# erwincoumans/tiny-differentiable-simulator

Hardware: AMD Instinct MI355X
Metric: env-steps/sec (higher is better)
Workload: dtype f64

## Files before the change

### tiny-differentiable-simulator_amd/csrc/tds_oct.hip

```cpp
#include <hip/hip_runtime.h>
#include <stdlib.h>

#include "tds_device_model.h"
#include "tds_kernels.h"
#include "tds_lanes.h"
#include "tds_step_shared.h"

#ifdef TDS_OCT_PROF
#ifndef TDS_OCT_PROF_WG
#define TDS_OCT_PROF_WG 3
#endif
__device__ unsigned long long tds_oct_prof_buf[32];
__device__ unsigned long long tds_oct_prof_clk[64];
__device__ unsigned long long tds_oct_prof_wg[3 * 2048];
__device__ int tds_oct_prof_iter = 500;
#define OCT_STAMP(k, pin)                                                                       \
  do {                                                                                          \
    unsigned long long t_;                                                                      \
    auto p_ = (pin);        \
    asm volatile("s_memtime %0\n\ts_waitcnt lgkmcnt(0)" : "=s"(t_), "+v"(p_)::"memory");        \
    if (prof_on) prof_t[k] = t_;                                                                \
  } while (0)
#else
#define OCT_STAMP(k, pin) do { } while (0)
// ... 28 lines not shown
__device__ __forceinline__ T pair_other(T v) { return oct_dpp<0xB1>(v); }
template <int K, typename T>
__device__ __forceinline__ T pair_bcast(T v) { return oct_dpp<(K == 0 ? 0xA0 : 0xF5)>(v); }
template <typename T>
__device__ __forceinline__ T oct_sum(T v) {
  asm volatile("" : "+v"(v));
  v += oct_dpp<0xB1>(v);
  v += oct_dpp<0x4E>(v);
  v += oct_dpp<0x141>(v);
  return v;
}
template <int K>
__device__ __forceinline__ double oct_bcast(double v) {
  const double t = __builtin_amdgcn_update_dpp(0.0, v, 0x150 + K, 0xF, 0x3, false);
  return __builtin_amdgcn_update_dpp(t, v, 0x150 + 8 + K, 0xF, 0xC, false);
}
template <int K>
__device__ __forceinline__ float oct_bcast(float v) {
  const int b = __float_as_int(v);
  const int t = __builtin_amdgcn_update_dpp(0, b, 0x150 + K, 0xF, 0x3, false);
  return __int_as_float(__builtin_amdgcn_update_dpp(t, b, 0x150 + 8 + K, 0xF, 0xC, false));
}

struct OctOff {
  int lcw, legf, swl, qdp, fac, win, xs, cp, stride;
};
struct OctLds {
  static constexpr int LCW = 6;
  static constexpr int ZW = 14;
  static constexpr int Z_B = 10, Z_A = 11, Z_G = 12, Z_HL = 13;
  static constexpr int NCP = 17;
};
__host__ __device__ inline OctOff oct_layout(int in_dim) {
  OctOff o;
  int at = in_dim + 4;
  at = (at + 1) & ~1;
  o.lcw = at;  at += 8 * OctLds::LCW;
  o.legf = at; at += 4 * 3;
  o.swl = at;  at += 8 * 6;
  o.qdp = at;  at += 8;
  o.fac = at;  at += 28;
  o.win = at;  at += 2 * 8 * OctLds::ZW;
  o.xs = at;   at += 3 * OctLds::NCP + 1;
  o.cp = at;   at += 5 * OctLds::NCP + 1;
  at = (at + 1) & ~1;
  while ((((at * 2) & 63) % 8) != 0 || ((at * 2) & 63) == 0 || ((at * 2) & 63) == 32) at += 2;
  o.stride = at;
  return o;
}

struct OctKernArgs {
  const void *mdl, *x_in;
  void *y_out;
  const void *actions;
  void *x_feedback, *obs_out;
  TdsStepCtl ctl;
  int n_envs;
  OctOff O;
};
using TB = TdsOctTab;

#ifdef TDS_OCT_NT
#define OCT_ST(v, p) __builtin_nontemporal_store((v), (p))
// ... 93 lines not shown
    unsigned long long c0_, c1_;
    asm volatile("s_memtime %0\n\ts_memrealtime %1\n\ts_waitcnt lgkmcnt(0)" : "=s"(c0_), "=s"(c1_)::"memory");
    tds_oct_prof_clk[2 * it] = c0_;
    tds_oct_prof_clk[2 * it + 1] = c1_;
  }
#endif
  const int lane = tid & 7;
  const int grp = (tid & 63) >> 3;
  const int env = blockIdx.x * 8 + grp;
  const bool valid = env < n_envs;
  T *const E = sm + grp * O.stride;
  T *const xr = E;
  const int leg = lane >> 1, pos = lane & 1;
  const int dq = 6 + lane;
  const T *const CL = CT + lane * TB::LSTR;
  typename TdsCtlRef<LOOP>::type ctl = TdsCtlRef<LOOP>::get(ctl_arg, ka_seg + __builtin_offsetof(OctKernArgs, ctl));
  const T dt = CT[TB::SC + TB::DT];
  const int pgs_iters = (int)CT[TB::SC + TB::PGS_ITERATIONS];
  const bool last = it == nsteps - 1;
  OCT_STAMP(0, tid);

  T q, qd, tau;
  T Sl[6], R[9], p[3], sw[6], v[6], a0[6];
  T R5[9], P[3], A4[3], A5[3], pA3[3], pA4[3], pA5[3], v5[6], a5[6];
  T Lc[6], l10, id0, id1, sq0, sq1, my_id, my_sq, Ls[15], ids[6], sq_ids[6], qd_new, qdr_new[6];
  T Cb, Cr[6], It[10];
  T u = T(0), urm = T(0);
  T u_init = T(0), urm_init = T(0);
  int na = 0, NA = 0;

  auto root_frame = [&](T sx, T cx, T sy, T cy, T sz, T cz) {
    R5[0] = cy * cz;                 R5[1] = -cy * sz;                R5[2] = sy;
    R5[3] = sx * sy * cz + cx * sz;  R5[4] = cx * cz - sx * sy * sz;  R5[5] = -sx * cy;
    R5[6] = sx * sz - cx * sy * cz;  R5[7] = cx * sy * sz + sx * cz;  R5[8] = cx * cy;
    P[0] = xr[0] + CT[TB::SC + TB::BASE_T];
    P[1] = xr[1] + CT[TB::SC + TB::BASE_T + 1];
    P[2] = xr[2] + CT[TB::SC + TB::BASE_T + 2];
    A4[0] = T(0); A4[1] = cx; A4[2] = sx;
    A5[0] = sy; A5[1] = -sx * cy; A5[2] = cx * cy;
    pA3[0] = T(0); pA3[1] = P[2]; pA3[2] = -P[1];
    cross3(P, A4, pA4);
    cross3(P, A5, pA5);
  };
  auto times_inertia = [&](const T *I, const T *s, T *F) {
    T t3[3];
    sym3_mulv(I, s, F);
    cross3(I + 6, s + 3, t3);
    F[0] += t3[0];
    F[1] += t3[1];
    F[2] += t3[2];
    cross3(I + 6, s, t3);
    F[3] = I[9] * s[3] - t3[0];
    F[4] = I[9] * s[4] - t3[1];
    F[5] = I[9] * s[5] - t3[2];
  };
  auto dot6 = [&](const T *a, const T *b) -> T { return dot3(a, b) + dot3(a + 3, b + 3); };

  auto main_kin = [&]() {
    OCT_MARK("main_top");
    q = xr[dq];
    qd = xr[nq + dq];
    tau = T(0);
    {
      const int act_i = act_slot;
      if (act_i >= 0) {
        const int var = nq + nd + adim;
        const T kp = xr[var], kd = xr[var + 1], max_force = xr[var + 2];
        const T act_lim = CT[TB::SC + TB::ACTION_LIMIT];
        T a = xr[nq + nd + act_i];
        a = a < act_lim ? a : act_lim;
        a = a > -act_lim ? a : -act_lim;
        const T q_des = CL[TB::IPOSE] + a;
        T f = kp * (q_des - q) + kd * (T(0) - qd);
        f = f > -max_force ? f : -max_force;
        f = f < max_force ? f : max_force;
        tau = f;
      }
      tau -= CL[TB::STIFF] * q + CL[TB::DAMP] * qd;
      asm volatile("" : "+v"(tau));
    }
    OCT_MARK("main_jcalc");
#pragma unroll
    for (int k = 0; k < 6; ++k) Sl[k] = CL[TB::S + k];
    T Rp[9], tp[3];
    {
      T sn, cs;
      tds_sincos(q * CL[TB::ROTF], &sn, &cs);
      const T c1 = T(1) - cs;
      const T nx = CL[TB::NAX], ny = CL[TB::NAX + 1], nz = CL[TB::NAX + 2];
      T RJ[9];
      RJ[0] = cs + c1 * CL[TB::NN + 0];
      RJ[1] = c1 * CL[TB::NN + 1] - sn * nz;
      RJ[2] = c1 * CL[TB::NN + 2] + sn * ny;
      RJ[3] = c1 * CL[TB::NN + 1] + sn * nz;
      RJ[4] = cs + c1 * CL[TB::NN + 3];
      RJ[5] = c1 * CL[TB::NN + 4] - sn * nx;
      RJ[6] = c1 * CL[TB::NN + 2] - sn * ny;
      RJ[7] = c1 * CL[TB::NN + 4] + sn * nx;
      RJ[8] = cs + c1 * CL[TB::NN + 5];
      const T tJ[3] = {Sl[3] * q, Sl[4] * q, Sl[5] * q};
      if (CT[TB::SC + TB::XT_IDENT] != T(0)) {
#pragma unroll
        for (int k = 0; k < 9; ++k) Rp[k] = RJ[k];
#pragma unroll
        for (int k = 0; k < 3; ++k) tp[k] = CL[TB::XT + 9 + k] + tJ[k];
      } else {
        T RT[9], r[3];
#pragma unroll
        for (int k = 0; k < 9; ++k) RT[k] = CL[TB::XT + k];
        mat3_mul(RT, RJ, Rp);
        mat3_mulv(RT, tJ, r);
#pragma unroll
        for (int k = 0; k < 3; ++k) tp[k] = CL[TB::XT + 9 + k] + r[k];
      }
    }
    OCT_MARK("main_rootsincos");
    {
      T rs, rc;
      tds_sincos(xr[3 + (lane < 3 ? lane : 0)], &rs, &rc);
      const T sx = oct_bcast<0>(rs), cx = oct_bcast<0>(rc);
      const T sy = oct_bcast<1>(rs), cy = oct_bcast<1>(rc);
      const T sz = oct_bcast<2>(rs), cz = oct_bcast<2>(rc);
      if constexpr (W2) {
        if (lane < 3) {
          T *const sc = E + O.win + 8 * OctLds::ZW + 96;
          sc[2 * lane] = rs;
          sc[2 * lane + 1] = rc;
        }
      }
      root_frame(sx, cx, sy, cy, sz, cz);
    }
    OCT_MARK("main_rootvel");
    {
      const T d0 = xr[nq + 0], d1 = xr[nq + 1], d2 = xr[nq + 2], d3 = xr[nq + 3], d4 = xr[nq + 4], d5 = xr[nq + 5];
      const T U[3] = {d0, d1, d2};
      const T J3[3] = {d3, T(0), T(0)}, J4[3] = {A4[0] * d4, A4[1] * d4, A4[2] * d4}, J5[3] = {A5[0] * d5, A5[1] * d5, A5[2] * d5};
      const T W4[3] = {J3[0] + J4[0], J3[1] + J4[1], J3[2] + J4[2]};
      const T W5[3] = {W4[0] + J5[0], W4[1] + J5[1], W4[2] + J5[2]};
      T pJ3[3], pJ4[3], pJ5[3];
      cross3(P, J3, pJ3);
      cross3(P, J4, pJ4);
      cross3(P, J5, pJ5);
      const T pW4[3] = {pJ3[0] + pJ4[0], pJ3[1] + pJ4[1], pJ3[2] + pJ4[2]};
      const T pW5[3] = {pW4[0] + pJ5[0], pW4[1] + pJ5[1], pW4[2] + pJ5[2]};
      const T V3[3] = {U[0] + pJ3[0], U[1] + pJ3[1], U[2] + pJ3[2]};
      const T V4[3] = {U[0] + pW4[0], U[1] + pW4[1], U[2] + pW4[2]};
      const T V5[3] = {U[0] + pW5[0], U[1] + pW5[1], U[2] + pW5[2]};
      T a45[3], a55[3], t1[3], t2[3], l3[3], l4[3], l5[3];
      cross3(J3, J4, a45);
      cross3(W4, J5, a55);
      cross3(J3, pJ3, t1);
      cross3(V3, J3, t2);
      l3[0] = t1[0] + t2[0]; l3[1] = t1[1] + t2[1]; l3[2] = t1[2] + t2[2];
      cross3(W4, pJ4, t1);
      cross3(V4, J4, t2);
      l4[0] = t1[0] + t2[0]; l4[1] = t1[1] + t2[1]; l4[2] = t1[2] + t2[2];
      cross3(W5, pJ5, t1);
      cross3(V5, J5, t2);
      l5[0] = t1[0] + t2[0]; l5[1] = t1[1] + t2[1]; l5[2] = t1[2] + t2[2];
#pragma unroll
      for (int k = 0; k < 3; ++k) {
        v5[k] = W5[k];
        v5[3 + k] = V5[k];
        a5[k] = a45[k] + a55[k];
        a5[3 + k] = (l3[k] + l4[k] + l5[k]) - CT[TB::SC + TB::GRAV + k];
      }
    }
    OCT_MARK("main_legs");
    {
      const bool take = pos == 1;
      T Rq[9], pq[3];
#pragma unroll
      for (int k = 0; k < 9; ++k) {
        const T sh = pair_bcast<0>(Rp[k]);
        Rq[k] = take ? sh : ((k == 0 || k == 4 || k == 8) ? T(1) : T(0));
      }
#pragma unroll
      for (int k = 0; k < 3; ++k) {
        const T sh = pair_bcast<0>(tp[k]);
        pq[k] = take ? sh : T(0);
      }
      T Rl[9], pl[3], r[3];
      mat3_mul(Rq, Rp, Rl);
      mat3_mulv(Rq, tp, r);
#pragma unroll
      for (int k = 0; k < 3; ++k) pl[k] = pq[k] + r[k];
      mat3_mul(R5, Rl, R);
      mat3_mulv(R5, pl, r);
      p[0] = P[0] + r[0];
      p[1] = P[1] + r[1];
      p[2] = P[2] + r[2];
      mat3_mulv(R, Sl, sw);
      mat3_mulv(R, Sl + 3, sw + 3);
      T c[3];
      cross3(p, sw, c);
      sw[3] += c[0];
      sw[4] += c[1];
      sw[5] += c[2];
      T vJ[6];
#pragma unroll
      for (int k = 0; k < 6; ++k) vJ[k] = sw[k] * qd;
#pragma unroll
      for (int k = 0; k < 6; ++k) {
        const T sh = pair_bcast<0>(vJ[k]);
        v[k] = v5[k] + (vJ[k] + (take ? sh : T(0)));
      }
      T cb[6];
      cross3(v, vJ, cb);
      T c1[3], c2[3];
      cross3(v, vJ + 3, c1);
      cross3(v + 3, vJ, c2);
      cb[3] = c1[0] + c2[0];
      cb[4] = c1[1] + c2[1];
      cb[5] = c1[2] + c2[2];
#pragma unroll
      for (int k = 0; k < 6; ++k) {
        const T sh = pair_bcast<0>(cb[k]);
        a0[k] = a5[k] + (cb[k] + (take ? sh : T(0)));
      }
    }
    OCT_MARK("main_publish_kin");
    {
      T *const swl = E + O.swl + lane * 6;
#pragma unroll
      for (int k = 0; k < 6; ++k) swl[k] = sw[k];
      if constexpr (W2) {
        T *const kin = E + O.win + 8 * OctLds::ZW + lane * 12;
#pragma unroll
        for (int k = 0; k < 9; ++k) kin[k] = R[k];
#pragma unroll
        for (int k = 0; k < 3; ++k) kin[9 + k] = p[k];
      }
    }
    OCT_MARK("main_kin_end");
    OCT_STAMP(1, sw[5]);
  };

// ... 20 lines not shown
  auto help_np = [&]() {
    OCT_MARK("help_np");
    if constexpr (LOOP) {
      if (it > 0 && ctl.obs_ring != nullptr && ctl.peer_arrive != nullptr)
        sig_tok = tds_peer_count_in(ctl, (o_slot == 0 ? ctl.obs_slots : o_slot) - 1);
      if (ctl.act_pool != nullptr && it + 1 < nsteps && valid)
        next_act = (T)tds_global((const TR *)ctl.act_pool)[((size_t)act_blk * ctl.act_envs + env) * adim + lane];
    }
    if constexpr (W2) {
      const T *const kin = E + O.win + 8 * OctLds::ZW + lane * 12;
#pragma unroll
      for (int k = 0; k < 9; ++k) R[k] = kin[k];
#pragma unroll
      for (int k = 0; k < 3; ++k) p[k] = kin[9 + k];
      const T *const sc = E + O.win + 8 * OctLds::ZW + 96;
      root_frame(sc[0], sc[1], sc[2], sc[3], sc[4], sc[5]);
    }
    {
      T *const cpx = E + O.cp;
      const T n[3] = {CT[TB::SC + TB::PLANE_N], CT[TB::SC + TB::PLANE_N + 1], CT[TB::SC + TB::PLANE_N + 2]};
      const T pc = CT[TB::SC + TB::PLANE_C];
      auto sphere = [&](const T *Rl, const T *pl, const T *loc, T rad, T *pt, T &dist) {
        T ctr[3];
        mat3_mulv(Rl, loc, ctr);
        ctr[0] += pl[0];
        ctr[1] += pl[1];
        ctr[2] += pl[2];
        const T t = -((-dot3(ctr, n)) + pc);
        dist = t - rad;
        pt[0] = ctr[0] - rad * n[0];
        pt[1] = ctr[1] - rad * n[1];
        pt[2] = ctr[2] - rad * n[2];
      };
      T pt0[3], pt1[3], ptt[3], d0, d1, dtt;
      sphere(R, p, CL + TB::CPL0, CL[TB::CPR0], pt0, d0);
      sphere(R, p, CL + TB::CPL1, CL[TB::CPR1], pt1, d1);
      sphere(R5, P, CT + TB::ROOT + TB::R_CPL, CT[TB::ROOT + TB::R_CPR], ptt, dtt);
      const bool act0 = valid && d0 < T(0), act1 = valid && d1 < T(0), actt = valid && dtt < T(0) && CT[TB::ROOT + TB::R_CPR] >= T(0);
      const unsigned long long b0 = __ballot(act0), b1 = __ballot(act1), bt = __ballot(actt);
      const unsigned m0 = (unsigned)((b0 >> (grp * 8)) & 0xFFull), m1 = (unsigned)((b1 >> (grp * 8)) & 0xFFull);
      const unsigned below = (1u << lane) - 1u;
      const int r0 = (actt ? 1 : 0) + __popc(m0 & below) + __popc(m1 & below);
      const int r1 = r0 + (act0 ? 1 : 0);
      if (act0) {
        cpx[0 * OctLds::NCP + r0] = pt0[0];
        cpx[1 * OctLds::NCP + r0] = pt0[1];
        cpx[2 * OctLds::NCP + r0] = pt0[2];
        cpx[3 * OctLds::NCP + r0] = d0;
        cpx[4 * OctLds::NCP + r0] = (T)lane;
      }
// ... 3 lines not shown
        cpx[2 * OctLds::NCP + r1] = pt1[2];
        cpx[3 * OctLds::NCP + r1] = d1;
        cpx[4 * OctLds::NCP + r1] = (T)lane;
      }
      if (actt && lane == 0) {
        cpx[0 * OctLds::NCP] = ptt[0];
        cpx[1 * OctLds::NCP] = ptt[1];
        cpx[2 * OctLds::NCP] = ptt[2];
        cpx[3 * OctLds::NCP] = dtt;
        cpx[4 * OctLds::NCP] = T(8);
      }
      na = (actt ? 1 : 0) + __popc(m0) + __popc(m1);
#pragma unroll
      for (int g = 0; g < 8; ++g) {
        const int c = __popc((unsigned)((b0 >> (g * 8)) & 0xFFull)) + __popc((unsigned)((b1 >> (g * 8)) & 0xFFull)) + (int)((bt >> (g * 8)) & 1ull);
        NA = c > NA ? c : NA;
      }
      if constexpr (W2) {
        if ((tid & 63) == 0) sm[in_dim + 3] = (T)NA;
      }
    }
    OCT_STAMP(8, na);
  };
  auto help_poses = [&]() {
    OCT_MARK("help_signal_poses");
    if constexpr (LOOP) {
      if (ctl.act_pool != nullptr && !last) xr[nq + nd + lane] = next_act;
      if (it > 0 && ctl.obs_ring != nullptr) {
        if (ctl.peer_arrive != nullptr) tds_peer_finish(ctl, (o_slot == 0 ? ctl.obs_slots : o_slot) - 1, sig_tok);
        else tds_signal_slot(ctl, (o_slot == 0 ? ctl.obs_slots : o_slot) - 1);
      }
    }
    TR *yo, *yo2;
    int yend, yend2;
    y_where(yo, yo2, yend, yend2);
    (void)yend;
    (void)yend2;
    if (valid && yo != nullptr && nv > 0) {
      auto pose_out = [&](const T *Rl, const T *pl, const T *vx, int k) {
        T Ro[9], po[3], qo[4];
        mat3_mul(Rl, vx, Ro);
        mat3_mulv(Rl, vx + 9, po);
        matrix_to_quat(Ro, qo);
        TR *o = yo + (nq + nd) + 7 * k;
        OCT_ST((TR)(pl[0] + po[0]), &o[0]);
        OCT_ST((TR)(pl[1] + po[1]), &o[1]);
        OCT_ST((TR)(pl[2] + po[2]), &o[2]);
        OCT_ST((TR)qo[0], &o[3]);
        OCT_ST((TR)qo[1], &o[4]);
        OCT_ST((TR)qo[2], &o[5]);
        OCT_ST((TR)qo[3], &o[6]);
        if (yo2 != nullptr) {
          TR *o2 = yo2 + (nq + nd) + 7 * k;
          OCT_ST((TR)(pl[0] + po[0]), &o2[0]);
          OCT_ST((TR)(pl[1] + po[1]), &o2[1]);
          OCT_ST((TR)(pl[2] + po[2]), &o2[2]);
          OCT_ST((TR)qo[0], &o2[3]);
          OCT_ST((TR)qo[1], &o2[4]);
          OCT_ST((TR)qo[2], &o2[5]);
          OCT_ST((TR)qo[3], &o2[6]);
        }
      };
      pose_out(R, p, CL + TB::VIS, 1 + lane);
      if (lane == 7) pose_out(R5, P, CT + TB::ROOT + TB::R_VIS, 0);
    }
    OCT_MARK("help_np_end");
    OCT_STAMP(9, na);
  };

  auto main_dyn = [&]() {
    auto rigid = [&](const T *Rl, const T *pl, T m, const T *com, const T *Ib, const T *vl, const T *al, T *Ic, T *fc) {
      T cw[3];
      mat3_mulv(Rl, com, cw);
      cw[0] += pl[0];
      cw[1] += pl[1];
      cw[2] += pl[2];
      T RI[9], Iw[9];
      mat3_mul(Rl, Ib, RI);
#pragma unroll
      for (int r = 0; r < 3; ++r)
#pragma unroll
        for (int c = 0; c < 3; ++c) Iw[3 * r + c] = RI[3 * r] * Rl[3 * c] + RI[3 * r + 1] * Rl[3 * c + 1] + RI[3 * r + 2] * Rl[3 * c + 2];
      const T c2 = dot3(cw, cw);
      Ic[0] = Iw[0] + m * (c2 - cw[0] * cw[0]);
      Ic[1] = T(0.5) * (Iw[1] + Iw[3]) - m * cw[0] * cw[1];
      Ic[2] = T(0.5) * (Iw[2] + Iw[6]) - m * cw[0] * cw[2];
      Ic[3] = Iw[4] + m * (c2 - cw[1] * cw[1]);
      Ic[4] = T(0.5) * (Iw[5] + Iw[7]) - m * cw[1] * cw[2];
      Ic[5] = Iw[8] + m * (c2 - cw[2] * cw[2]);
      Ic[6] = m * cw[0];
      Ic[7] = m * cw[1];
      Ic[8] = m * cw[2];
      Ic[9] = m;
      const T *const h = Ic + 6;
      T Iv[6], Ia[6], t3[3];
      sym3_mulv(Ic, vl, Iv);
      cross3(h, vl + 3, t3);
      Iv[0] += t3[0];
      Iv[1] += t3[1];
      Iv[2] += t3[2];
      cross3(h, vl, t3);
      Iv[3] = m * vl[3] - t3[0];
      Iv[4] = m * vl[4] - t3[1];
      Iv[5] = m * vl[5] - t3[2];
      sym3_mulv(Ic, al, Ia);
      cross3(h, al + 3, t3);
      Ia[0] += t3[0];
      Ia[1] += t3[1];
      Ia[2] += t3[2];
      cross3(h, al, t3);
      Ia[3] = m * al[3] - t3[0];
      Ia[4] = m * al[4] - t3[1];
      Ia[5] = m * al[5] - t3[2];
      T u3[3];
      cross3(vl, Iv, fc);
      cross3(vl + 3, Iv + 3, u3);
      fc[0] += u3[0];
      fc[1] += u3[1];
      fc[2] += u3[2];
      cross3(vl, Iv + 3, fc + 3);
#pragma unroll
      for (int k = 0; k < 6; ++k) fc[k] += Ia[k];
    };
    OCT_MARK("main_rigid");
    T Ic[10], fc[6];
    rigid(R, p, CL[TB::MASS], CL + TB::COM, CL + TB::INER, v, a0, Ic, fc);
    T ft[6];
    rigid(R5, P, CT[TB::ROOT + TB::R_MASS], CT + TB::ROOT + TB::R_COM, CT + TB::ROOT + TB::R_INER, v5, a5, It, ft);
    OCT_STAMP(2, ft[5]);
    OCT_MARK("main_totals");
#pragma unroll
    for (int k = 0; k < 10; ++k) It[k] += oct_sum(Ic[k]);
#pragma unroll
    for (int k = 0; k < 6; ++k) ft[k] += oct_sum(fc[k]);
    {
      const T recv = pos == 0 ? T(1) : T(0);
#pragma unroll
      for (int k = 0; k < 6; ++k) fc[k] += recv * pair_bcast<1>(fc[k]);
#pragma unroll
      for (int k = 0; k < 10; ++k) Ic[k] += recv * pair_bcast<1>(Ic[k]);
    }
    OCT_MARK("main_FC");
    T Fc[6];
    times_inertia(Ic, sw, Fc);
    Cb = dot6(sw, fc);
    const T ax3[6] = {T(1), T(0), T(0), pA3[0], pA3[1], pA3[2]}, ax4[6] = {A4[0], A4[1], A4[2], pA4[0], pA4[1], pA4[2]},
            ax5[6] = {A5[0], A5[1], A5[2], pA5[0], pA5[1], pA5[2]};
    Cr[0] = ft[3];
    Cr[1] = ft[4];
    Cr[2] = ft[5];
    Cr[3] = dot6(ax3, ft);
    Cr[4] = dot6(ax4, ft);
    Cr[5] = dot6(ax5, ft);
    T Bm0, Bm1, Cc[6];
    {
      T s0[6];
#pragma unroll
      for (int k = 0; k < 6; ++k) s0[k] = pair_bcast<0>(sw[k]);
      Bm0 = dot6(Fc, s0);
      Bm1 = dot6(Fc, sw);
      Cc[0] = Fc[3];
      Cc[1] = Fc[4];
      Cc[2] = Fc[5];
      Cc[3] = dot6(Fc, ax3);
      Cc[4] = dot6(Fc, ax4);
      Cc[5] = dot6(Fc, ax5);
    }
    OCT_MARK("main_legldl");
    {
      const T b00 = pair_bcast<0>(Bm0);
      const T b10 = pair_bcast<1>(Bm0), b11 = pair_bcast<1>(Bm1);
      sq0 = rsqrt_full<T>(b00);
      id0 = sq0 * sq0;
      l10 = b10 * id0;
      sq1 = rsqrt_full<T>(b11 - l10 * b10);
      id1 = sq1 * sq1;
    }
    my_id = pos == 0 ? id0 : id1;
    my_sq = pos == 0 ? sq0 : sq1;
    {
      T W[6];
      const T m1 = pos == 1 ? l10 : T(0);
#pragma unroll
      for (int r = 0; r < 6; ++r) {
        W[r] = Cc[r] - m1 * pair_bcast<0>(Cc[r]);
        Lc[r] = W[r] * my_id;
      }
      T *const lcw = E + O.lcw + lane * OctLds::LCW;
      T *const wl = E + O.xs + lane * 6;
// ... 3 lines not shown
        wl[r] = W[r];
      }
      if (pos == 0) {
        T *const lf = E + O.legf + leg * 3;
        lf[0] = l10;
        lf[1] = sq0;
        lf[2] = sq1;
      }
    }
    OCT_STAMP(3, Lc[5]);
  };
  auto main_dyn2 = [&]() {
    OCT_MARK("main_schur");
    {
      const T *const lcw = E + O.lcw;
      const T *const wl = E + O.xs;
      T *const Ssum = E + O.fac;
      const int code = (int)CL[TB::SCHUR];
#pragma unroll
      for (int pass = 0; pass < 3; ++pass) {
        const int rc = (code >> (6 * pass)) & 63;
        const int r = rc >> 3, rp = rc & 7;
        const int e = (r * (r + 1)) / 2 + rp;
        T acc = T(0);
#pragma unroll
        for (int l = 0; l < 8; ++l) acc += lcw[l * OctLds::LCW + r] * wl[l * 6 + rp];
        Ssum[e] = acc;
      }
    }
    OCT_MARK("main_Rblock");
    const T ax3[6] = {T(1), T(0), T(0), pA3[0], pA3[1], pA3[2]}, ax4[6] = {A4[0], A4[1], A4[2], pA4[0], pA4[1], pA4[2]},
            ax5[6] = {A5[0], A5[1], A5[2], pA5[0], pA5[1], pA5[2]};
    T Sm[21];
    {
      const T m = It[9];
      T F3[6], F4[6], F5[6];
      times_inertia(It, ax3, F3);
      times_inertia(It, ax4, F4);
      times_inertia(It, ax5, F5);
      Sm[0] = m;
      Sm[1] = T(0); Sm[2] = m;
      Sm[3] = T(0); Sm[4] = T(0); Sm[5] = m;
      Sm[6] = F3[3]; Sm[7] = F3[4]; Sm[8] = F3[5]; Sm[9] = dot6(ax3, F3);
      Sm[10] = F4[3]; Sm[11] = F4[4]; Sm[12] = F4[5]; Sm[13] = dot6(ax4, F3); Sm[14] = dot6(ax4, F4);
      Sm[15] = F5[3]; Sm[16] = F5[4]; Sm[17] = F5[5]; Sm[18] = dot6(ax5, F3); Sm[19] = dot6(ax5, F4); Sm[20] = dot6(ax5, F5);
    }
    OCT_SYNC();
    OCT_MARK("main_ldl6");
    {
      const T *const Ssum = E + O.fac;
#pragma unroll
      for (int e = 0; e < 21; ++e) Sm[e] -= Ssum[e];
      static_for<0, 6>([&](auto kc) {
        constexpr int k = decltype(kc)::value;
        const T rs = rsqrt_full<T>(Sm[(k * (k + 1)) / 2 + k]);
        const T inv = rs * rs;
        sq_ids[k] = rs;
        ids[k] = inv;
        T col[6];
        static_for<k + 1, 6>([&](auto rc) {
          constexpr int r = decltype(rc)::value;
          col[r] = Sm[(r * (r + 1)) / 2 + k];
          Ls[(r * (r - 1)) / 2 + k] = col[r] * inv;
        });
        static_for<k + 1, 6>([&](auto rc) {
          constexpr int r = decltype(rc)::value;
          static_for<k + 1, r + 1>([&](auto cc) {
            constexpr int c = decltype(cc)::value;
            Sm[(r * (r + 1)) / 2 + c] -= Ls[(r * (r - 1)) / 2 + k] * col[c];
          });
        });
      });
    }
    OCT_STAMP(4, Ls[14]);
    OCT_MARK("main_fd");
// ... 57 lines not shown
      const T dist = cpx[3 * OctLds::NCP + ac];
      const T owner = cpx[4 * OctLds::NCP + ac];
      const T *const dir = CT + TB::SC + TB::NB + 3 * tk;
      const T e[3] = {dir[0], dir[1], dir[2]};
      const int ol = real ? (int)owner : 8;
      const bool on_leg = ol < 8;
      const int hl = on_leg ? (ol & ~1) : 0;
      const bool ank = on_leg && (ol & 1);
      T sh[6], sa[6];
#pragma unroll
      for (int c = 0; c < 6; ++c) {
        sh[c] = swl[hl * 6 + c];
        sa[c] = swl[(hl + 1) * 6 + c];
      }
      const T qh = xr[nq + 6 + hl], qa = xr[nq + 6 + hl + 1];
      T mo[3];
      cross3(Pc, e, mo);
      const T j0 = dot3(e, sh + 3) + dot3(mo, sh), j1 = dot3(e, sa + 3) + dot3(mo, sa);
      const T z0 = on_leg ? j0 : T(0), z1 = ank ? j1 : T(0);
      T zr[6];
      zr[0] = e[0];
      zr[1] = e[1];
      zr[2] = e[2];
      zr[3] = dot3(e, pA3) + mo[0];
      zr[4] = dot3(e, pA4) + dot3(mo, A4);
      zr[5] = dot3(e, pA5) + dot3(mo, A5);
      const T vrow = ((z0 * qh + z1 * qa) + (zr[0] * xr[nq + 0] + zr[1] * xr[nq + 1])) +
                     ((zr[2] * xr[nq + 2] + zr[3] * xr[nq + 3]) + (zr[4] * xr[nq + 4] + zr[5] * xr[nq + 5]));
      const T crow = tk == 0 ? (T(1) + CT[TB::SC + TB::RESTITUTION]) * vrow - CT[TB::SC + TB::ERP_OVER_DT] * dist : vrow;
      row[0] = z0;
      row[1] = z1;
#pragma unroll
      for (int rr = 0; rr < 6; ++rr) row[2 + rr] = real ? zr[rr] : T(0);
      row[8] = T(0);
      row[9] = T(0);
      row[OctLds::Z_B] = real ? crow : T(0);
      row[OctLds::Z_A] = real ? T(1) : T(0);
      row[OctLds::Z_HL] = on_leg ? (T)hl : T(-2);
      OCT_MARK("rows_geom_end");
  };
  auto rows_leg = [&](int wi) {
      OCT_MARK("rows_leg");
      T *const row = E + O.win + (wi & 1) * (8 * OctLds::ZW) + lane * OctLds::ZW;
      const T *const lcw = E + O.lcw;
      T z0 = row[0], z1 = row[1], zr[6];
#pragma unroll
      for (int rr = 0; rr < 6; ++rr) zr[rr] = row[2 + rr];
      const T hlv = row[OctLds::Z_HL];
// ... 384 lines not shown
    } else {
      OCT_BAR();
      help_np();
      if (NA > 0) rows_geom(0);
      OCT_BAR();
      if (NA > 0) rows_leg(0);
      help_poses();
      OCT_BAR();
      const int nw = windows();
      if (nw > 0) {
        if constexpr (TDS_OCT_PRIO == 2) __builtin_amdgcn_s_setprio(3);
        help_get_factors();
        rows_root(0);
        if constexpr (TDS_OCT_PRIO == 2) __builtin_amdgcn_s_setprio(0);
      }
      for (int wi = 0; wi < nw; ++wi) {
        if (wi > 0) {
          rows_geom(wi);
          rows_leg(wi);
          rows_root(wi);
        }
        OCT_BAR();
      }
      OCT_BAR();
      help_rec();
    }
  } else {
    main_kin();
    OCT_SYNC();
    help_np();
    help_poses();
    main_dyn();
    OCT_SYNC();
    main_dyn2();
    main_fd();
    const int nw = windows();
    for (int wi = 0; wi < nw; ++wi) {
      rows_geom(wi);
      rows_leg(wi);
      rows_root(wi);
      OCT_SYNC();
      main_sweep(wi);
    }
    main_fin();
    main_pool();
    OCT_SYNC();
    help_rec();
    if constexpr (LOOP) OCT_SYNC();
  }
#ifdef TDS_OCT_PROF
  if (prof_on && (tid & 63) == 0) {
#pragma unroll
    for (int k = 16; k < 24; ++k)
      if (is_main) tds_oct_prof_buf[k] = prof_t[k];
#pragma unroll
    for (int k = 0; k < 14; ++k)
      if (((k < 8 || k >= 12) && is_main) || (k >= 8 && k < 12 && is_help)) tds_oct_prof_buf[k] = prof_t[k];
    if (is_help) tds_oct_prof_buf[15] = (unsigned long long)NA;
  }
#endif
  if constexpr (LOOP) {
    act_blk = act_blk + 1 >= ctl_arg.act_blocks ? 0 : act_blk + 1;
    y_slot = y_slot + 1 >= ctl_arg.y_slots ? 0 : y_slot + 1;
    o_slot = o_slot + 1 >= ctl_arg.obs_slots ? 0 : o_slot + 1;
  }
  }
#ifdef TDS_OCT_PROF
  if (threadIdx.x == 0 && blockIdx.x < 2048) {
    unsigned long long c_;
    asm volatile("s_waitcnt vmcnt(0)\n\ts_memrealtime %0\n\ts_waitcnt lgkmcnt(0)" : "=s"(c_)::"memory");
    tds_oct_prof_wg[3 * blockIdx.x + 2] = c_;
  }
#endif
}

template <typename T, typename TR, bool LOOP, int BUILD>
__global__ __launch_bounds__(BUILD >= 2 ? 128 : 64) __attribute__((amdgpu_waves_per_eu(BUILD == 2 ? 2 : 1, BUILD == 2 ? 2 : 1)))
void tds_oct_kernel(const DevModel<T> *__restrict__ mdl_arg, const TR *x_in, TR *__restrict__ y_out,
                    const TR *__restrict__ actions, TR *x_feedback, TR *__restrict__ obs_out, TdsStepCtl ctl_arg, int n_envs,
                    OctOff O) {
// ... 65 lines not shown
```

Baseline: 590.8 million.

## Specialize root-axis algebra, fuse small vector ops, defer root pose output

Exploits the known sparsity of the root joint axes (zero entries in the ax3/ax4 motion vectors) to expand the inertia products, cross products and dot products by hand, dropping multiplies by zero and several temporaries. Small matrix-vector, cross and dot helpers are fused into add/sum variants so they form chained FMA expressions. The root-link pose quaternion output moves out of help_poses into a later help_root_pose, which rebuilds the rotation from sin/cos values stashed in LDS, and the quaternion conversion becomes branchless with selects. This cuts ALU work and register pressure on the critical main path, at the cost of an extra LDS region and a slightly different floating-point evaluation order.

```diff
diff --git a/tiny-differentiable-simulator_amd/csrc/tds_oct.hip b/tiny-differentiable-simulator_amd/csrc/tds_oct.hip
--- a/tiny-differentiable-simulator_amd/csrc/tds_oct.hip
+++ b/tiny-differentiable-simulator_amd/csrc/tds_oct.hip
@@ -74,8 +74,71 @@
   return __int_as_float(__builtin_amdgcn_update_dpp(t, b, 0x150 + 8 + K, 0xF, 0xC, false));
 }
 
+template <typename T>
+__device__ __forceinline__ void mat3_mulv_add(const T *m, const T *v, const T *t, T *o) {
+  const T x = t[0] + m[0] * v[0] + m[1] * v[1] + m[2] * v[2];
+  const T y = t[1] + m[3] * v[0] + m[4] * v[1] + m[5] * v[2];
+  const T z = t[2] + m[6] * v[0] + m[7] * v[1] + m[8] * v[2];
+  o[0] = x;
+  o[1] = y;
+  o[2] = z;
+}
+template <typename T>
+__device__ __forceinline__ void cross3_add(const T *a, const T *b, const T *t, T *o) {
+  const T x = t[0] + a[1] * b[2] - a[2] * b[1];
+  const T y = t[1] + a[2] * b[0] - a[0] * b[2];
+  const T z = t[2] + a[0] * b[1] - a[1] * b[0];
+  o[0] = x;
+  o[1] = y;
+  o[2] = z;
+}
+template <typename T>
+__device__ __forceinline__ void cross3_sum(const T *a, const T *b, const T *c, const T *d, T *o) {
+  const T x = a[1] * b[2] - a[2] * b[1] + c[1] * d[2] - c[2] * d[1];
+  const T y = a[2] * b[0] - a[0] * b[2] + c[2] * d[0] - c[0] * d[2];
+  const T z = a[0] * b[1] - a[1] * b[0] + c[0] * d[1] - c[1] * d[0];
+  o[0] = x;
+  o[1] = y;
+  o[2] = z;
+}
+template <typename T>
+__device__ __forceinline__ void sym3_mulv_cross(const T *s, const T *v, const T *a, const T *b, T *o) {
+  const T x = s[0] * v[0] + s[1] * v[1] + s[2] * v[2] + a[1] * b[2] - a[2] * b[1];
+  const T y = s[1] * v[0] + s[3] * v[1] + s[4] * v[2] + a[2] * b[0] - a[0] * b[2];
+  const T z = s[2] * v[0] + s[4] * v[1] + s[5] * v[2] + a[0] * b[1] - a[1] * b[0];
+  o[0] = x;
+  o[1] = y;
+  o[2] = z;
+}
+template <typename T>
+__device__ __forceinline__ T dot6_chain(const T *a, const T *b) {
+  return a[0] * b[0] + a[1] * b[1] + a[2] * b[2] + a[3] * b[3] + a[4] * b[4] + a[5] * b[5];
+}
+template <typename T>
+__device__ __forceinline__ void matrix_to_quat_sel(const T *m, T *q) {
+  const T trace = m[0] + m[4] + m[8];
+  const bool neg = trace < T(0);
+  const int i = m[0] < m[4] ? (m[4] < m[8] ? 2 : 1) : (m[0] < m[8] ? 2 : 0);
+  const bool i0 = i == 0, i1 = i == 1;
+  const T a0 = ((m[0] - m[4]) - m[8]) + T(1), a1 = ((m[4] - m[8]) - m[0]) + T(1), a2 = ((m[8] - m[0]) - m[4]) + T(1);
+  const T a_ = neg ? (i0 ? a0 : i1 ? a1 : a2) : trace + T(1);
+  const T r_ = rsqrt_full<T>(a_);
+  const T th = a_ * r_ * T(0.5);
+  const T s = T(0.5) * r_;
+  const T d0 = m[5] - m[7], d1 = m[6] - m[2], d2 = m[1] - m[3];
+  const T s01 = m[1] + m[3], s02 = m[2] + m[6], s12 = m[5] + m[7];
+  const T x0 = (neg ? (i1 ? s01 : s02) : d0) * s;
+  const T x1 = (neg ? (i0 ? s01 : s12) : d1) * s;
+  const T x2 = (neg ? (i0 ? s02 : s12) : d2) * s;
+  const T x3 = (i0 ? d0 : i1 ? d1 : d2) * s;
+  q[0] = neg && i0 ? th : x0;
+  q[1] = neg && i1 ? th : x1;
+  q[2] = neg && !i0 && !i1 ? th : x2;
+  q[3] = -(neg ? x3 : th);
+}
+
 struct OctOff {
-  int lcw, legf, swl, qdp, fac, win, xs, cp, stride;
+  int lcw, legf, swl, rootf, fac, win, xs, cp, stride;
 };
 struct OctLds {
   static constexpr int LCW = 6;
@@ -90,7 +153,7 @@
   o.lcw = at;  at += 8 * OctLds::LCW;
   o.legf = at; at += 4 * 3;
   o.swl = at;  at += 8 * 6;
-  o.qdp = at;  at += 8;
+  o.rootf = at; at += 10;
   o.fac = at;  at += 28;
   o.win = at;  at += 2 * 8 * OctLds::ZW;
   o.xs = at;   at += 3 * OctLds::NCP + 1;
@@ -230,39 +293,42 @@
 
   T q, qd, tau;
   T Sl[6], R[9], p[3], sw[6], v[6], a0[6];
-  T R5[9], P[3], A4[3], A5[3], pA3[3], pA4[3], pA5[3], v5[6], a5[6];
+  T R5[9], P[3], A4[3], A5[3], pA4[3], pA5[3], v5[6], a5[6];
   T Lc[6], l10, id0, id1, sq0, sq1, my_id, my_sq, Ls[15], ids[6], sq_ids[6], qd_new, qdr_new[6];
   T Cb, Cr[6], It[10];
   T u = T(0), urm = T(0);
   T u_init = T(0), urm_init = T(0);
   int na = 0, NA = 0;
 
+  auto root_rot = [&](T sx, T cx, T sy, T cy, T sz, T cz, T *Rr) {
+    Rr[0] = cy * cz;                 Rr[1] = -cy * sz;                Rr[2] = sy;
+    Rr[3] = sx * sy * cz + cx * sz;  Rr[4] = cx * cz - sx * sy * sz;  Rr[5] = -sx * cy;
+    Rr[6] = sx * sz - cx * sy * cz;  Rr[7] = cx * sy * sz + sx * cz;  Rr[8] = cx * cy;
+  };
   auto root_frame = [&](T sx, T cx, T sy, T cy, T sz, T cz) {
-    R5[0] = cy * cz;                 R5[1] = -cy * sz;                R5[2] = sy;
-    R5[3] = sx * sy * cz + cx * sz;  R5[4] = cx * cz - sx * sy * sz;  R5[5] = -sx * cy;
-    R5[6] = sx * sz - cx * sy * cz;  R5[7] = cx * sy * sz + sx * cz;  R5[8] = cx * cy;
+    root_rot(sx, cx, sy, cy, sz, cz, R5);
     P[0] = xr[0] + CT[TB::SC + TB::BASE_T];
     P[1] = xr[1] + CT[TB::SC + TB::BASE_T + 1];
     P[2] = xr[2] + CT[TB::SC + TB::BASE_T + 2];
     A4[0] = T(0); A4[1] = cx; A4[2] = sx;
     A5[0] = sy; A5[1] = -sx * cy; A5[2] = cx * cy;
-    pA3[0] = T(0); pA3[1] = P[2]; pA3[2] = -P[1];
-    cross3(P, A4, pA4);
+    pA4[0] = P[1] * sx - P[2] * cx;
+    pA4[1] = -(P[0] * sx);
+    pA4[2] = P[0] * cx;
     cross3(P, A5, pA5);
   };
+  auto dot_ax3 = [&](const T *f) -> T { return f[0] + P[2] * f[4] - P[1] * f[5]; };
+  auto dot_ax4 = [&](const T *f) -> T { return A4[1] * f[1] + A4[2] * f[2] + pA4[0] * f[3] + pA4[1] * f[4] + pA4[2] * f[5]; };
+  auto dot_ax5 = [&](const T *f) -> T { return A5[0] * f[0] + A5[1] * f[1] + A5[2] * f[2] + pA5[0] * f[3] + pA5[1] * f[4] + pA5[2] * f[5]; };
   auto times_inertia = [&](const T *I, const T *s, T *F) {
     T t3[3];
-    sym3_mulv(I, s, F);
-    cross3(I + 6, s + 3, t3);
-    F[0] += t3[0];
-    F[1] += t3[1];
-    F[2] += t3[2];
+    sym3_mulv_cross(I, s, I + 6, s + 3, F);
     cross3(I + 6, s, t3);
     F[3] = I[9] * s[3] - t3[0];
     F[4] = I[9] * s[4] - t3[1];
     F[5] = I[9] * s[5] - t3[2];
   };
-  auto dot6 = [&](const T *a, const T *b) -> T { return dot3(a, b) + dot3(a + 3, b + 3); };
+  auto dot6 = [&](const T *a, const T *b) -> T { return dot6_chain(a, b); };
 
   auto main_kin = [&]() {
     OCT_MARK("main_top");
@@ -306,20 +372,18 @@
       RJ[6] = c1 * CL[TB::NN + 2] - sn * ny;
       RJ[7] = c1 * CL[TB::NN + 4] + sn * nx;
       RJ[8] = cs + c1 * CL[TB::NN + 5];
-      const T tJ[3] = {Sl[3] * q, Sl[4] * q, Sl[5] * q};
       if (CT[TB::SC + TB::XT_IDENT] != T(0)) {
 #pragma unroll
         for (int k = 0; k < 9; ++k) Rp[k] = RJ[k];
 #pragma unroll
-        for (int k = 0; k < 3; ++k) tp[k] = CL[TB::XT + 9 + k] + tJ[k];
+        for (int k = 0; k < 3; ++k) tp[k] = CL[TB::XT + 9 + k] + Sl[3 + k] * q;
       } else {
-        T RT[9], r[3];
+        const T tJ[3] = {Sl[3] * q, Sl[4] * q, Sl[5] * q};
+        T RT[9];
 #pragma unroll
         for (int k = 0; k < 9; ++k) RT[k] = CL[TB::XT + k];
         mat3_mul(RT, RJ, Rp);
-        mat3_mulv(RT, tJ, r);
-#pragma unroll
-        for (int k = 0; k < 3; ++k) tp[k] = CL[TB::XT + 9 + k] + r[k];
+        mat3_mulv_add(RT, tJ, CL + TB::XT + 9, tp);
       }
     }
     OCT_MARK("main_rootsincos");
@@ -329,8 +393,12 @@
       const T sx = oct_bcast<0>(rs), cx = oct_bcast<0>(rc);
       const T sy = oct_bcast<1>(rs), cy = oct_bcast<1>(rc);
       const T sz = oct_bcast<2>(rs), cz = oct_bcast<2>(rc);
-      if constexpr (W2) {
-        if (lane < 3) {
+      if (lane < 3) {
+        T *const rf = E + O.rootf;
+        rf[2 * lane] = rs;
+        rf[2 * lane + 1] = rc;
+        rf[6 + lane] = xr[lane] + CT[TB::SC + TB::BASE_T + lane];
+        if constexpr (W2) {
           T *const sc = E + O.win + 8 * OctLds::ZW + 96;
           sc[2 * lane] = rs;
           sc[2 * lane + 1] = rc;
@@ -342,36 +410,32 @@
     {
       const T d0 = xr[nq + 0], d1 = xr[nq + 1], d2 = xr[nq + 2], d3 = xr[nq + 3], d4 = xr[nq + 4], d5 = xr[nq + 5];
       const T U[3] = {d0, d1, d2};
-      const T J3[3] = {d3, T(0), T(0)}, J4[3] = {A4[0] * d4, A4[1] * d4, A4[2] * d4}, J5[3] = {A5[0] * d5, A5[1] * d5, A5[2] * d5};
-      const T W4[3] = {J3[0] + J4[0], J3[1] + J4[1], J3[2] + J4[2]};
+      const T J4y = A4[1] * d4, J4z = A4[2] * d4;
+      const T J5[3] = {A5[0] * d5, A5[1] * d5, A5[2] * d5};
+      const T W4[3] = {d3, J4y, J4z};
       const T W5[3] = {W4[0] + J5[0], W4[1] + J5[1], W4[2] + J5[2]};
-      T pJ3[3], pJ4[3], pJ5[3];
-      cross3(P, J3, pJ3);
-      cross3(P, J4, pJ4);
+      const T pJ3y = P[2] * d3, pJ3z = -(P[1] * d3);
+      const T pJ4[3] = {P[1] * J4z - P[2] * J4y, -(P[0] * J4z), P[0] * J4y};
+      T pJ5[3];
       cross3(P, J5, pJ5);
-      const T pW4[3] = {pJ3[0] + pJ4[0], pJ3[1] + pJ4[1], pJ3[2] + pJ4[2]};
+      const T pW4[3] = {pJ4[0], pJ3y + pJ4[1], pJ3z + pJ4[2]};
       const T pW5[3] = {pW4[0] + pJ5[0], pW4[1] + pJ5[1], pW4[2] + pJ5[2]};
-      const T V3[3] = {U[0] + pJ3[0], U[1] + pJ3[1], U[2] + pJ3[2]};
+      const T V3y = U[1] + pJ3y, V3z = U[2] + pJ3z;
       const T V4[3] = {U[0] + pW4[0], U[1] + pW4[1], U[2] + pW4[2]};
       const T V5[3] = {U[0] + pW5[0], U[1] + pW5[1], U[2] + pW5[2]};
-      T a45[3], a55[3], t1[3], t2[3], l3[3], l4[3], l5[3];
-      cross3(J3, J4, a45);
-      cross3(W4, J5, a55);
-      cross3(J3, pJ3, t1);
-      cross3(V3, J3, t2);
-      l3[0] = t1[0] + t2[0]; l3[1] = t1[1] + t2[1]; l3[2] = t1[2] + t2[2];
-      cross3(W4, pJ4, t1);
-      cross3(V4, J4, t2);
-      l4[0] = t1[0] + t2[0]; l4[1] = t1[1] + t2[1]; l4[2] = t1[2] + t2[2];
-      cross3(W5, pJ5, t1);
-      cross3(V5, J5, t2);
-      l5[0] = t1[0] + t2[0]; l5[1] = t1[1] + t2[1]; l5[2] = t1[2] + t2[2];
+      const T a45[3] = {W4[1] * J5[2] - W4[2] * J5[1], W4[2] * J5[0] - W4[0] * J5[2] - d3 * J4z, W4[0] * J5[1] - W4[1] * J5[0] + d3 * J4y};
+      const T l3y = V3z * d3 - d3 * pJ3z, l3z = d3 * pJ3y - V3y * d3;
+      const T l4[3] = {W4[1] * pJ4[2] - W4[2] * pJ4[1] + V4[1] * J4z - V4[2] * J4y, W4[2] * pJ4[0] - W4[0] * pJ4[2] - V4[0] * J4z,
+                       W4[0] * pJ4[1] - W4[1] * pJ4[0] + V4[0] * J4y};
+      T l5[3];
+      cross3_sum(W5, pJ5, V5, J5, l5);
+      const T lsum[3] = {l4[0] + l5[0], l3y + l4[1] + l5[1], l3z + l4[2] + l5[2]};
 #pragma unroll
       for (int k = 0; k < 3; ++k) {
         v5[k] = W5[k];
         v5[3 + k] = V5[k];
-        a5[k] = a45[k] + a55[k];
-        a5[3 + k] = (l3[k] + l4[k] + l5[k]) - CT[TB::SC + TB::GRAV + k];
+        a5[k] = a45[k];
+        a5[3 + k] = lsum[k] - CT[TB::SC + TB::GRAV + k];
       }
     }
     OCT_MARK("main_legs");
@@ -388,23 +452,17 @@
         const T sh = pair_bcast<0>(tp[k]);
         pq[k] = take ? sh : T(0);
       }
-      T Rl[9], pl[3], r[3];
+      T Rl[9], pl[3];
       mat3_mul(Rq, Rp, Rl);
-      mat3_mulv(Rq, tp, r);
-#pragma unroll
-      for (int k = 0; k < 3; ++k) pl[k] = pq[k] + r[k];
+      mat3_mulv_add(Rq, tp, pq, pl);
       mat3_mul(R5, Rl, R);
-      mat3_mulv(R5, pl, r);
-      p[0] = P[0] + r[0];
-      p[1] = P[1] + r[1];
-      p[2] = P[2] + r[2];
+      mat3_mulv_add(R5, pl, P, p);
       mat3_mulv(R, Sl, sw);
-      mat3_mulv(R, Sl + 3, sw + 3);
-      T c[3];
-      cross3(p, sw, c);
-      sw[3] += c[0];
-      sw[4] += c[1];
-      sw[5] += c[2];
+      {
+        T rl[3];
+        mat3_mulv(R, Sl + 3, rl);
+        cross3_add(p, sw, rl, sw + 3);
+      }
       T vJ[6];
 #pragma unroll
       for (int k = 0; k < 6; ++k) vJ[k] = sw[k] * qd;
@@ -415,12 +473,7 @@
       }
       T cb[6];
       cross3(v, vJ, cb);
-      T c1[3], c2[3];
-      cross3(v, vJ + 3, c1);
-      cross3(v + 3, vJ, c2);
-      cb[3] = c1[0] + c2[0];
-      cb[4] = c1[1] + c2[1];
-      cb[5] = c1[2] + c2[2];
+      cross3_sum(v, vJ + 3, v + 3, vJ, cb + 3);
 #pragma unroll
       for (int k = 0; k < 6; ++k) {
         const T sh = pair_bcast<0>(cb[k]);
@@ -487,10 +540,7 @@
       const T pc = CT[TB::SC + TB::PLANE_C];
       auto sphere = [&](const T *Rl, const T *pl, const T *loc, T rad, T *pt, T &dist) {
         T ctr[3];
-        mat3_mulv(Rl, loc, ctr);
-        ctr[0] += pl[0];
-        ctr[1] += pl[1];
-        ctr[2] += pl[2];
+        mat3_mulv_add(Rl, loc, pl, ctr);
         const T t = -((-dot3(ctr, n)) + pc);
         dist = t - rad;
         pt[0] = ctr[0] - rad * n[0];
@@ -540,6 +590,47 @@
     }
     OCT_STAMP(8, na);
   };
+  auto pose_out = [&](TR *yo, TR *yo2, const T *Rl, const T *pl, const T *vx, int k) {
+    T Ro[9], po[3], qo[4];
+    mat3_mul(Rl, vx, Ro);
+    mat3_mulv_add(Rl, vx + 9, pl, po);
+    matrix_to_quat_sel(Ro, qo);
+    TR *o = yo + (nq + nd) + 7 * k;
+    OCT_ST((TR)po[0], &o[0]);
+    OCT_ST((TR)po[1], &o[1]);
+    OCT_ST((TR)po[2], &o[2]);
+    OCT_ST((TR)qo[0], &o[3]);
+    OCT_ST((TR)qo[1], &o[4]);
+    OCT_ST((TR)qo[2], &o[5]);
+    OCT_ST((TR)qo[3], &o[6]);
+    if (yo2 != nullptr) {
+      TR *o2 = yo2 + (nq + nd) + 7 * k;
+      OCT_ST((TR)po[0], &o2[0]);
+      OCT_ST((TR)po[1], &o2[1]);
+      OCT_ST((TR)po[2], &o2[2]);
+      OCT_ST((TR)qo[0], &o2[3]);
+      OCT_ST((TR)qo[1], &o2[4]);
+      OCT_ST((TR)qo[2], &o2[5]);
+      OCT_ST((TR)qo[3], &o2[6]);
+    }
+  };
+  auto help_root_pose = [&]() {
+    OCT_MARK("help_root_pose");
+    TR *yo, *yo2;
+    int yend, yend2;
+    y_where(yo, yo2, yend, yend2);
+    (void)yend;
+    (void)yend2;
+    if (valid && yo != nullptr && nv > 0 && lane == 7) {
+      const T *const rf = E + O.rootf;
+      T Rr[9];
+      root_rot(rf[0], rf[1], rf[2], rf[3], rf[4], rf[5], Rr);
+      const T Pr[3] = {rf[6], rf[7], rf[8]};
+      pose_out(yo, yo2, Rr, Pr, CT + TB::ROOT + TB::R_VIS, 0);
+    }
+    OCT_MARK("help_root_pose_end");
+    OCT_STAMP(14, na);
+  };
   auto help_poses = [&]() {
     OCT_MARK("help_signal_poses");
     if constexpr (LOOP) {
@@ -554,34 +645,7 @@
     y_where(yo, yo2, yend, yend2);
     (void)yend;
     (void)yend2;
-    if (valid && yo != nullptr && nv > 0) {
-      auto pose_out = [&](const T *Rl, const T *pl, const T *vx, int k) {
-        T Ro[9], po[3], qo[4];
-        mat3_mul(Rl, vx, Ro);
-        mat3_mulv(Rl, vx + 9, po);
-        matrix_to_quat(Ro, qo);
-        TR *o = yo + (nq + nd) + 7 * k;
-        OCT_ST((TR)(pl[0] + po[0]), &o[0]);
-        OCT_ST((TR)(pl[1] + po[1]), &o[1]);
-        OCT_ST((TR)(pl[2] + po[2]), &o[2]);
-        OCT_ST((TR)qo[0], &o[3]);
-        OCT_ST((TR)qo[1], &o[4]);
-        OCT_ST((TR)qo[2], &o[5]);
-        OCT_ST((TR)qo[3], &o[6]);
-        if (yo2 != nullptr) {
-          TR *o2 = yo2 + (nq + nd) + 7 * k;
-          OCT_ST((TR)(pl[0] + po[0]), &o2[0]);
-          OCT_ST((TR)(pl[1] + po[1]), &o2[1]);
-          OCT_ST((TR)(pl[2] + po[2]), &o2[2]);
-          OCT_ST((TR)qo[0], &o2[3]);
-          OCT_ST((TR)qo[1], &o2[4]);
-          OCT_ST((TR)qo[2], &o2[5]);
-          OCT_ST((TR)qo[3], &o2[6]);
-        }
-      };
-      pose_out(R, p, CL + TB::VIS, 1 + lane);
-      if (lane == 7) pose_out(R5, P, CT + TB::ROOT + TB::R_VIS, 0);
-    }
+    if (valid && yo != nullptr && nv > 0) pose_out(yo, yo2, R, p, CL + TB::VIS, 1 + lane);
     OCT_MARK("help_np_end");
     OCT_STAMP(9, na);
   };
@@ -589,10 +653,7 @@
   auto main_dyn = [&]() {
     auto rigid = [&](const T *Rl, const T *pl, T m, const T *com, const T *Ib, const T *vl, const T *al, T *Ic, T *fc) {
       T cw[3];
-      mat3_mulv(Rl, com, cw);
-      cw[0] += pl[0];
-      cw[1] += pl[1];
-      cw[2] += pl[2];
+      mat3_mulv_add(Rl, com, pl, cw);
       T RI[9], Iw[9];
       mat3_mul(Rl, Ib, RI);
 #pragma unroll
@@ -612,33 +673,22 @@
       Ic[9] = m;
       const T *const h = Ic + 6;
       T Iv[6], Ia[6], t3[3];
-      sym3_mulv(Ic, vl, Iv);
-      cross3(h, vl + 3, t3);
-      Iv[0] += t3[0];
-      Iv[1] += t3[1];
-      Iv[2] += t3[2];
+      sym3_mulv_cross(Ic, vl, h, vl + 3, Iv);
       cross3(h, vl, t3);
       Iv[3] = m * vl[3] - t3[0];
       Iv[4] = m * vl[4] - t3[1];
       Iv[5] = m * vl[5] - t3[2];
-      sym3_mulv(Ic, al, Ia);
-      cross3(h, al + 3, t3);
-      Ia[0] += t3[0];
-      Ia[1] += t3[1];
-      Ia[2] += t3[2];
+      sym3_mulv_cross(Ic, al, h, al + 3, Ia);
       cross3(h, al, t3);
       Ia[3] = m * al[3] - t3[0];
       Ia[4] = m * al[4] - t3[1];
       Ia[5] = m * al[5] - t3[2];
-      T u3[3];
-      cross3(vl, Iv, fc);
-      cross3(vl + 3, Iv + 3, u3);
-      fc[0] += u3[0];
-      fc[1] += u3[1];
-      fc[2] += u3[2];
-      cross3(vl, Iv + 3, fc + 3);
-#pragma unroll
-      for (int k = 0; k < 6; ++k) fc[k] += Ia[k];
+      {
+        T u3[3];
+        cross3_add(vl, Iv, Ia, u3);
+        cross3_add(vl + 3, Iv + 3, u3, fc);
+        cross3_add(vl, Iv + 3, Ia + 3, fc + 3);
+      }
     };
     OCT_MARK("main_rigid");
     T Ic[10], fc[6];
@@ -648,9 +698,16 @@
     OCT_STAMP(2, ft[5]);
     OCT_MARK("main_totals");
 #pragma unroll
+    for (int k = 0; k < 6; ++k) ft[k] += oct_sum(fc[k]);
+    Cr[0] = ft[3];
+    Cr[1] = ft[4];
+    Cr[2] = ft[5];
+    Cr[3] = dot_ax3(ft);
+    Cr[4] = dot_ax4(ft);
+    Cr[5] = dot_ax5(ft);
+    asm volatile("" : "+v"(Cr[3]), "+v"(Cr[4]), "+v"(Cr[5]));
+#pragma unroll
     for (int k = 0; k < 10; ++k) It[k] += oct_sum(Ic[k]);
-#pragma unroll
-    for (int k = 0; k < 6; ++k) ft[k] += oct_sum(fc[k]);
     {
       const T recv = pos == 0 ? T(1) : T(0);
 #pragma unroll
@@ -662,14 +719,6 @@
     T Fc[6];
     times_inertia(Ic, sw, Fc);
     Cb = dot6(sw, fc);
-    const T ax3[6] = {T(1), T(0), T(0), pA3[0], pA3[1], pA3[2]}, ax4[6] = {A4[0], A4[1], A4[2], pA4[0], pA4[1], pA4[2]},
-            ax5[6] = {A5[0], A5[1], A5[2], pA5[0], pA5[1], pA5[2]};
-    Cr[0] = ft[3];
-    Cr[1] = ft[4];
-    Cr[2] = ft[5];
-    Cr[3] = dot6(ax3, ft);
-    Cr[4] = dot6(ax4, ft);
-    Cr[5] = dot6(ax5, ft);
     T Bm0, Bm1, Cc[6];
     {
       T s0[6];
@@ -680,9 +729,9 @@
       Cc[0] = Fc[3];
       Cc[1] = Fc[4];
       Cc[2] = Fc[5];
-      Cc[3] = dot6(Fc, ax3);
-      Cc[4] = dot6(Fc, ax4);
-      Cc[5] = dot6(Fc, ax5);
+      Cc[3] = dot_ax3(Fc);
+      Cc[4] = dot_ax4(Fc);
+      Cc[5] = dot_ax5(Fc);
     }
     OCT_MARK("main_legldl");
     {
@@ -732,35 +781,49 @@
         const int rc = (code >> (6 * pass)) & 63;
         const int r = rc >> 3, rp = rc & 7;
         const int e = (r * (r + 1)) / 2 + rp;
-        T acc = T(0);
-#pragma unroll
-        for (int l = 0; l < 8; ++l) acc += lcw[l * OctLds::LCW + r] * wl[l * 6 + rp];
+        T acc = lcw[r] * wl[rp];
+#pragma unroll
+        for (int l = 1; l < 8; ++l) acc += lcw[l * OctLds::LCW + r] * wl[l * 6 + rp];
         Ssum[e] = acc;
       }
     }
     OCT_MARK("main_Rblock");
-    const T ax3[6] = {T(1), T(0), T(0), pA3[0], pA3[1], pA3[2]}, ax4[6] = {A4[0], A4[1], A4[2], pA4[0], pA4[1], pA4[2]},
-            ax5[6] = {A5[0], A5[1], A5[2], pA5[0], pA5[1], pA5[2]};
+    const T ax5[6] = {A5[0], A5[1], A5[2], pA5[0], pA5[1], pA5[2]};
     T Sm[21];
     {
       const T m = It[9];
+      const T *const h = It + 6;
+      const T cx = A4[1], sx = A4[2];
       T F3[6], F4[6], F5[6];
-      times_inertia(It, ax3, F3);
-      times_inertia(It, ax4, F4);
+      F3[0] = It[0] - h[1] * P[1] - h[2] * P[2];
+      F3[1] = It[1] + h[0] * P[1];
+      F3[2] = It[2] + h[0] * P[2];
+      F3[4] = m * P[2] - h[2];
+      F3[5] = h[1] - m * P[1];
+      F4[0] = It[1] * cx + It[2] * sx + h[1] * pA4[2] - h[2] * pA4[1];
+      F4[1] = It[3] * cx + It[4] * sx + h[2] * pA4[0] - h[0] * pA4[2];
+      F4[2] = It[4] * cx + It[5] * sx + h[0] * pA4[1] - h[1] * pA4[0];
+      F4[3] = m * pA4[0] - (h[1] * sx - h[2] * cx);
+      F4[4] = m * pA4[1] + h[0] * sx;
+      F4[5] = m * pA4[2] - h[0] * cx;
       times_inertia(It, ax5, F5);
       Sm[0] = m;
       Sm[1] = T(0); Sm[2] = m;
       Sm[3] = T(0); Sm[4] = T(0); Sm[5] = m;
-      Sm[6] = F3[3]; Sm[7] = F3[4]; Sm[8] = F3[5]; Sm[9] = dot6(ax3, F3);
-      Sm[10] = F4[3]; Sm[11] = F4[4]; Sm[12] = F4[5]; Sm[13] = dot6(ax4, F3); Sm[14] = dot6(ax4, F4);
-      Sm[15] = F5[3]; Sm[16] = F5[4]; Sm[17] = F5[5]; Sm[18] = dot6(ax5, F3); Sm[19] = dot6(ax5, F4); Sm[20] = dot6(ax5, F5);
+      Sm[6] = T(0); Sm[7] = F3[4]; Sm[8] = F3[5]; Sm[9] = F3[0] + P[2] * F3[4] - P[1] * F3[5];
+      Sm[10] = F4[3]; Sm[11] = F4[4]; Sm[12] = F4[5];
+      Sm[13] = cx * F3[1] + sx * F3[2] + pA4[1] * F3[4] + pA4[2] * F3[5];
+      Sm[14] = dot_ax4(F4);
+      Sm[15] = F5[3]; Sm[16] = F5[4]; Sm[17] = F5[5];
+      Sm[18] = A5[0] * F3[0] + A5[1] * F3[1] + A5[2] * F3[2] + pA5[1] * F3[4] + pA5[2] * F3[5];
+      Sm[19] = dot_ax5(F4); Sm[20] = dot_ax5(F5);
     }
     OCT_SYNC();
     OCT_MARK("main_ldl6");
     {
       const T *const Ssum = E + O.fac;
 #pragma unroll
-      for (int e = 0; e < 21; ++e) Sm[e] -= Ssum[e];
+      for (int e = 0; e < 21; ++e) Sm[e] = (e == 1 || e == 3 || e == 4 || e == 6) ? -Ssum[e] : Sm[e] - Ssum[e];
       static_for<0, 6>([&](auto kc) {
         constexpr int k = decltype(kc)::value;
         const T rs = rsqrt_full<T>(Sm[(k * (k + 1)) / 2 + k]);
@@ -864,8 +927,8 @@
       zr[0] = e[0];
       zr[1] = e[1];
       zr[2] = e[2];
-      zr[3] = dot3(e, pA3) + mo[0];
-      zr[4] = dot3(e, pA4) + dot3(mo, A4);
+      zr[3] = e[1] * P[2] - e[2] * P[1] + mo[0];
+      zr[4] = dot3(e, pA4) + mo[1] * A4[1] + mo[2] * A4[2];
       zr[5] = dot3(e, pA5) + dot3(mo, A5);
       const T vrow = ((z0 * qh + z1 * qa) + (zr[0] * xr[nq + 0] + zr[1] * xr[nq + 1])) +
                      ((zr[2] * xr[nq + 2] + zr[3] * xr[nq + 3]) + (zr[4] * xr[nq + 4] + zr[5] * xr[nq + 5]));
@@ -1296,6 +1359,7 @@
         }
         OCT_BAR();
       }
+      help_root_pose();
       OCT_BAR();
       help_rec();
     }
@@ -1316,6 +1380,7 @@
       OCT_SYNC();
       main_sweep(wi);
     }
+    help_root_pose();
     main_fin();
     main_pool();
     OCT_SYNC();
@@ -1330,6 +1395,7 @@
 #pragma unroll
     for (int k = 0; k < 14; ++k)
       if (((k < 8 || k >= 12) && is_main) || (k >= 8 && k < 12 && is_help)) tds_oct_prof_buf[k] = prof_t[k];
+    if (is_help) tds_oct_prof_buf[14] = prof_t[14];
     if (is_help) tds_oct_prof_buf[15] = (unsigned long long)NA;
   }
 #endif
```

After: 584.6 million. 1.1% lower.
